# Hyberge/GPUFluidSimulation

Measured on AMD Instinct MI355X. Metric: Mvoxels/s per step (bimocq3D rising smoke), higher is better.
Workload: dtype f32

## Files before the change

gpufluidsimulation_amd/_lib.py:

```python
import ctypes as C
import os

HERE = os.path.dirname(os.path.abspath(__file__))
HIP_SO = os.path.join(HERE, "libbimocq_hip.so")
HOST_SO = os.path.join(HERE, "libbimocq_host.so")

VP = C.c_void_p
c_f, c_i, c_b, c_d = C.c_float, C.c_int, C.c_bool, C.c_double

_G = [c_f, c_i, c_i, c_i]

HIP_SIGS = {
    "gpu_solve_forward": (None, [VP] * 6 + _G + [c_f, c_f]),
    "gpu_solve_backwardDMC": (None, [VP] * 9 + _G + [c_f]),
    "gpu_advect_velocity": (None, [VP] * 9 + _G + [c_b]),
    "gpu_advect_vel_double": (None, [VP] * 12 + _G + [c_b, c_f]),
    "gpu_advect_field": (None, [VP] * 5 + _G + [c_b]),
    "gpu_advect_field_double": (None, [VP] * 8 + _G + [c_b, c_f]),
    "gpu_advect_vel_double_global": (None, [VP] * 12 + _G + [c_b, c_f]),
    "gpu_advect_field_double_global": (None, [VP] * 8 + _G + [c_b, c_f]),
    "gpu_accumulate_velocity": (None, [VP] * 9 + _G + [c_b, c_f]),
    "gpu_accumulate_field": (None, [VP] * 5 + _G + [c_b, c_f]),
    "gpu_estimate_distortion": (None, [VP] * 7 + _G),
    "gpu_add": (None, [VP, VP, c_f, c_i]),
# ... 28 lines not shown
    "fl_aux_end": (None, []),
    "fl_aux_join": (None, []),
    "fl_malloc_host": (VP, [C.c_size_t]),
    "fl_free_host": (None, [VP]),
    "fl_download_begin": (VP, [VP, VP, C.c_size_t]),
    "fl_download_wait": (c_i, [VP]),
    "fl_event_create": (VP, []),
    "fl_event_record": (None, [VP]),
    "fl_event_elapsed_ms": (c_f, [VP, VP]),
    "fl_event_destroy": (None, [VP]),
    "fl_last_error": (c_i, []),
    "fl_last_error_string": (C.c_char_p, []),
    "fl_clear_error": (None, []),
    "fl_compute_stream": (VP, []),
    "fl_set_option": (None, [c_i, c_i]),
    "fl_get_option": (c_i, [c_i]),
    "fl_jacobi_profile": (None, [C.POINTER(c_d), C.POINTER(C.c_longlong), C.POINTER(C.c_longlong)]),
    "fl_jacobi_kernel_name": (C.c_char_p, []),
    "fl_mg_smooth_kernel_name": (C.c_char_p, []),
    "fl_mg_fused_launches": (C.c_longlong, []),
    "fl_mg_residual_launches": (C.c_longlong, []),
    "fl_sparse_stats": (None, [C.POINTER(C.c_longlong), c_i]),
    "fl_sparse_stats_kind": (None, [c_i, C.POINTER(C.c_longlong), c_i]),
    "gpu_brick_flags": (c_i, [VP, VP, c_i, c_i, c_i, VP, C.POINTER(c_i)]),
    "gpu_init_maps": (None, [VP, VP, VP] + _G),
    "gpu_maps_quarter_safe": (c_i, [VP, VP, VP] + _G),
    "fl_map_guard_reset": (None, [c_i]),
    "fl_map_guard_read": (None, [C.POINTER(c_i)]),
    "fl_nonfinite_seen": (c_i, [c_i]),
    "gpu_solve_forward_hint": (None, [VP] * 6 + _G + [c_f, c_f, C.c_uint]),
    "gpu_solve_backwardDMC_hint": (None, [VP] * 9 + _G + [c_f, C.c_uint]),
    "fl_map_kernel_name": (C.c_char_p, [c_i]),
    "fl_map_kernels_seen": (c_i, [c_i]),
    "gpu_max_abs3": (c_f, [VP, VP, VP, c_i, c_i, c_i]),
    "gpu_divergence": (None, [VP] * 4 + [c_i, c_i, c_i, c_f]),
    "gpu_jacobi_sweeps": (c_i, [VP, VP, VP, c_i, c_i, c_i, c_i, c_f, c_f]),
    "gpu_gradient": (None, [VP] * 4 + [c_i, c_i, c_i, c_f]),
    "fl_comm_selftest": (c_i, []),
    "gpu_diffuse_sweeps": (c_i, [VP, VP, VP, c_i, c_i, c_i, c_i, c_f]),
    "gpu_max_field": (c_f, [VP, C.c_size_t]),
    "gpu_max_field_owned": (c_f, [VP, c_i, c_i, c_i]),
    "gpu_map_travel_z": (None, [VP, VP, c_f, c_i, c_i, c_i, C.POINTER(c_f)]),
    "gpu_smoothing_jacobi": (None, [VP, VP, VP, c_d, c_d, c_i, c_i, c_i, c_i]),
    "gpu_mgcg_slab_supported": (c_i, [c_i] * 8),
    "gpu_multi_grid_conjugate_gradient_slab": (None, [VP, VP, VP, VP] + [c_i] * 7 + [c_d]),
    "gpu_gradient_delta": (None, [VP] * 7 + [c_i, c_i, c_i, c_f]),
# ... 70 lines not shown
    "gpu_sample_particles": (c_i, [VP, c_i, c_i, c_i, c_f, c_f, c_f, c_f, VP, VP, VP, VP, C.c_long]),
    "gpu_seed_particles": (c_i, [VP] * 3 + [c_i] * 7 + [C.c_uint] + _G),
    "gpu_sort_particles": (c_i, [VP] * 8 + [C.c_long] + _G),
}

FL_OK, FL_ERR_NO_DEVICE, FL_ERR_HIP, FL_ERR_BAD_ARGUMENT, FL_ERR_UNSUPPORTED, FL_ERR_COMM = range(6)
FL_OPT_RESIDUAL_STRIDE, FL_OPT_SKIP_UNIT_BLEND, FL_OPT_JACOBI_VARIANT = 1, 2, 3
FL_OPT_PROFILE_JACOBI, FL_OPT_JACOBI_KCHUNK, FL_OPT_JACOBI_ROWS, FL_OPT_STRUCTURED_MAPS = 4, 5, 6, 7
FL_OPT_JACOBI_FUSE, FL_OPT_JACOBI_KCHUNK2, FL_OPT_MGCG_GRAPH, FL_OPT_FAST_LERP = 8, 9, 10, 11
FL_OPT_FUSED_HOUSEKEEPING = 12
FL_OPT_MAP_QUARTER_FP32 = 13
FL_OPT_MGCG_TILE = 14
FL_MAP_HINT_FINITE, FL_MAP_HINT_IDENTITY = 1, 2
FL_OPT_PROFILE_COMM = 15
FL_OPT_RESERVE_CUS = 16
FL_OPT_MGCG_BOTTOM = 17
FL_OPT_MGCG_FUSE = 20
FL_OPT_FIELD_WINDOW = 18
FL_OPT_COMM_CHECK = 19
FL_OPT_SKIP_EMPTY_BRICKS = 21
FL_OPT_DIAG_KCHUNK = 22
FL_OPT_RENDER_KCHUNK = 23
FL_OPT_CONFINE_KCHUNK = 24
STAT_NAMES = ("e2", "m2", "d2", "div_max", "rho", "rho_i", "rho_j", "rho_k", "T", "vort_max")
STAT_COUNT = len(STAT_NAMES)
LOAD_NAMES = ("px", "py", "pz", "mx", "my", "mz", "faces", "psum")
LOAD_COUNT = len(LOAD_NAMES)
MAX_BOUNDARIES = 16


class BimocqLibraryMissing(RuntimeError):
    pass


_hip = None


def hip_lib():
    global _hip
    if _hip is None:
        if not os.path.exists(HIP_SO):
            raise BimocqLibraryMissing(
                f"{HIP_SO} not found: build it with `make` (or __graft_entry__.build()); "
                "there is no CPU fallback for the product path")
        lib = C.CDLL(HIP_SO)
        for name, (res, args) in HIP_SIGS.items():
# ... 20 lines not shown
```

gpufluidsimulation_amd/csrc/bq_advect.hip:

```cpp
#include "bq_device.hip.h"
#include "bq_gather_op.hip.h"
#include "bq_host.h"
#include "bq_launch_geom.h"
#include "bq_obstacle.hip.h"
#include "bq_sparse.hip.h"

#include <algorithm>
#include <cstdint>
#include <type_traits>
#include <vector>

namespace bq {
inline namespace BQ_VARIANT {

#define BQ_IJK(nbi, nbj, nbk)                                   \
    const int i = blockIdx.x * 64 + threadIdx.x;                \
    const int j = blockIdx.y * 4 + threadIdx.y;                 \
    const int k = blockIdx.z + g.kw0;                           \
    if (i >= (nbi) || j >= (nbj) || k >= (nbk)) return;         \
    const int kg = k + g.koff;                                  \
    (void)kg;

#define BQ_IJK_WINDOW(ilo, ihi, jlo, jhi, klo, khi) BQ_IJK_WINDOW_AT((int)blockIdx.x, (int)blockIdx.y, (int)blockIdx.z, ilo, ihi, jlo, jhi, klo, khi)
#define BQ_IJK_WINDOW_AT(bx_, by_, bz_, ilo, ihi, jlo, jhi, klo, khi)                         \
// ... 98 lines not shown
    f3 pn = mk3(dmc_axis(pt.x, vl.x, ax, substep), dmc_axis(pt.y, vl.y, ay, substep), dmc_axis(pt.z, vl.z, az, substep));
    f3 r;
    if constexpr (IDIN) r = map_at_identity<P2>(in, sp, pn, g.ni, g.nj, g.nk);
    else r = map_at<P2>(in, sp, pn);
    size_t id = (size_t)i + (size_t)g.ni * j + (size_t)g.ni * g.nj * k;
    xo[id] = r.x; yo[id] = r.y; zo[id] = r.z;
    guard_map_values(guard, r, sp.h);
}

template <bool P2, bool PT, int SD>
__device__ __forceinline__ void mapped9(const Map3 &m, const Spacing &sp, const Nine &n, f3 c, int i, int j, int kl, f3 out[9])
{
    if constexpr (P2 && !PT && SD >= 0) {
        map9<SD == 1, SD == 2, SD == 3>(m, i, j, kl, out);
    } else {
        if (!PT) {
#pragma unroll
            for (int ii = 0; ii < 8; ii++) out[ii] = map_at<P2>(m, sp, nine_corner(n, c, ii));
        }
        out[8] = map_at<P2>(m, sp, c);
    }
}

template <bool P2, bool PT, int NF, bool GE1>
__device__ __forceinline__ void blend9_gather_w(const Field (&src)[NF], const Spacing &sp, f3 org, const f3 (&mp)[9],
                                                const float (&w)[NF], float (&sum)[NF], float (&value)[NF])
{
    if (!PT) {
#pragma unroll
        for (int ii = 0; ii < 8; ii++) {
            const Cell c = locate<P2, true>(src[0], sp, org, mp[ii]);
#pragma unroll
            for (int f = 0; f < NF; f++) sum[f] += w[f] * gather<GE1>(src[f], c);
        }
    }
    const Cell c = locate<P2, true>(src[0], sp, org, mp[8]);
#pragma unroll
    for (int f = 0; f < NF; f++) {
        value[f] = gather<GE1>(src[f], c);
        if (PT) sum[f] += w[f] * value[f];
    }
}
template <bool P2, bool PT, int NF, bool GE1>
__device__ __forceinline__ void blend9_gather(const Field (&src)[NF], const Spacing &sp, f3 org, const f3 (&mp)[9],
                                              float (&sum)[NF], float (&value)[NF])
{
    float w[NF];
#pragma unroll
    for (int f = 0; f < NF; f++) w[f] = PT ? 1.0f : 0.125f;
    blend9_gather_w<P2, PT, NF, GE1>(src, sp, org, mp, w, sum, value);
}
template <bool PT>
__device__ __forceinline__ bool wave_all_ge(const f3 (&mp)[9], float h)
{
    float m = fminf(mp[8].x, fminf(mp[8].y, mp[8].z));
    if (!PT) {
#pragma unroll
        for (int a9 = 0; a9 < 8; a9++) m = fminf(m, fminf(mp[a9].x, fminf(mp[a9].y, mp[a9].z)));
    }
// ... 107 lines not shown
}

__global__ __launch_bounds__(256) void unit_blend_kernel(float *field, Grid g, int dx, int dy, int dz)
{
    const int nbi = g.ni + dx, nbj = g.nj + dy, nbk = g.nk + dz;
    BQ_IJK(nbi, nbj, nbk)
    if (!(2 + dx < i && i < nbi - 3 && 2 + dy < j && j < nbj - 3 && 2 + dz < kg && kg < g.nkg + dz - 3)) return;
    size_t id = (size_t)i + (size_t)nbi * j + (size_t)nbi * nbj * k;
    field[id] = field[id] + 0.0f;
}

template <bool P2, bool PT, int SD, int NF, bool ID, bool Q4 = false, int SPARSE = 0>
__global__ __launch_bounds__(256, NF == 1 ? 7 : 6) void cumulate_kernel(CumulateArgs<NF> a,
                                                       const float *mx, const float *my, const float *mz,
                                                       Spacing sp, Grid g, int dx, int dy, int dz, MapTabs tabs, Sparse sps)
{
    static_assert(!SPARSE || (SD == 0 && !ID && kStaged<P2, PT, SD>), "the skip exists for unstaggered staged launches only");
    using Op = GatherOp<kOpCumulate>;
    constexpr int m = Op::margin;
    const int nbi = g.ni + dx, nbj = g.nj + dy, nbk = g.nk + dz;
    int bX = blockIdx.x, bY = blockIdx.y, bZ = blockIdx.z;
    if constexpr (SPARSE == 1) { if (*sps.word != sps.epoch) return; }
    if constexpr (SPARSE == 2) { if (!listed_block(sps, bX, bY, bZ)) return; }
    BQ_IJK_WINDOW_AT(bX, bY, bZ, m + dx, nbi - m - 1, m + dy, nbj - m - 1, m + dz, g.nkg + dz - m - 1)
    if (block_out) return;
    const float h = sp.h;
    Map3 map{make_field(mx, g.ni, g.nj, g.nk, g.koff), make_field(my, g.ni, g.nj, g.nk, g.koff), make_field(mz, g.ni, g.nj, g.nk, g.koff)};
    Nine n = nine_setup(h, dx, dy, dz);
    f3 lo = Op::lo(h), hi = Op::hi(h, g.ni, g.nj, g.nkg);
    f3 c = nine_centre(n, i, j, kg);
    const size_t id = (size_t)i + (size_t)nbi * j + (size_t)nbi * nbj * k;
    __shared__ float tile[kStaged<P2, PT, SD> && !ID && SPARSE != 1 ? 3 * kTile : 32];
    (void)tabs; (void)sps;
    if constexpr (SPARSE == 1) {
        const Field mf[3] = {map.x, map.y, map.z};
        float mn[3], mxv[3]; bool bad;
        float dst_own[NF];
#pragma unroll
        for (int f = 0; f < NF; f++) dst_own[f] = active ? a.dst[f][id] : 0.f;
        tile_range(mf, i0, j0, k, tile, m, nbi - m - 1, m, nbj - m - 1, mn, mxv, bad);
        const bool skip = taps_in_empty_bricks<P2>(sps, mn, mxv, bad, lo, hi, sp, nbi, nbj, nbk);
        count_block(sps, skip);
        if (!skip) { list_block(sps, bX + gridDim.x * (bY + gridDim.y * bZ)); return; }
        if (!active) return;
#pragma unroll
        for (int f = 0; f < NF; f++) {
// ... 16 lines not shown
            float s9[9];
            map9_component<0, 0, 0>(src, i, j, k, s9);
            float sum = 0.f;
#pragma unroll
            for (int ii = 0; ii < 8; ii++) sum += Op::weight(false, coeff) * s9[ii];
            a.dst[f][id] += Op::result(sum, s9[8], coeff, 0.f);
        }
        return;
    }
    f3 mp[9];
    if constexpr (kStaged<P2, PT, SD>) {
        const Field mf[3] = {map.x, map.y, map.z};
        stage_tiles<3>(mf, i0, j0, k, tile);
        if (!active) return;
        if constexpr (P2) map9_lds<SD == 1, SD == 2, SD == 3, Q4>(tile, mp);
        else map9_lds_tab<SD == 1, SD == 2, SD == 3>(tile, tabs, i, j, kg, mp);
    } else {
        if (!active) return;
        mapped9<P2, PT, SD>(map, sp, n, c, i, j, k, mp);
    }
    const bool ge1 = NF == 1 && wave_all_ge<PT>(mp, h);
#pragma unroll
    for (int a9 = 0; a9 < 9; a9++) mp[a9] = clamp3_ordered(mp[a9], lo, hi);
    Field src[NF];
    float sum[NF], value[NF], w[NF];
#pragma unroll
    for (int f = 0; f < NF; f++) {
        src[f] = make_field(a.src[f], nbi, nbj, nbk, g.koff);
        sum[f] = 0.f;
        w[f] = Op::weight(PT, a.coeff[f]);
    }
    if (NF == 1 && ge1) blend9_gather_w<P2, PT, NF, true>(src, sp, n.org, mp, w, sum, value);
    else                blend9_gather_w<P2, PT, NF, false>(src, sp, n.org, mp, w, sum, value);
#pragma unroll
    for (int f = 0; f < NF; f++) {
        a.dst[f][id] += Op::result(sum[f], value[f], a.coeff[f], 0.f);
    }
}

template <bool P2, int SD>
__global__ __launch_bounds__(256) void wall_fixup_kernel(const float *src, int src_nk, int src_koff,
                                                         const float *before, float *dst,
                                                         const float *mx, const float *my, const float *mz,
                                                         Spacing sp, Grid g, int dx, int dy, int dz, float coeff,
                                                         int face_axis, int face_index, int kw1)
{
    const int nbi = g.ni + dx, nbj = g.nj + dy, nbk = g.nk + dz;
    const int a = blockIdx.x * 64 + threadIdx.x, b = blockIdx.y * 4 + threadIdx.y;
    int i, j, k;
    if (face_axis == 0)      { i = face_index; j = a; k = b + g.kw0; }
    else if (face_axis == 1) { i = a; j = face_index; k = b + g.kw0; }
    else                     { i = a; j = b; k = face_index - g.koff; }
    if (i >= nbi || j >= nbj || k < g.kw0 || k >= kw1 || k >= nbk) return;
    const int kg = k + g.koff;
    using Op = GatherOp<kOpCumulate>;
    constexpr int om = Op::margin;
// ... 403 lines not shown
        kchunk = 32;
        while (kchunk > 8 && (long)gx * gy * ((planes + kchunk - 1) / kchunk) < 3L * 4 * rt().num_cus) kchunk /= 2;
    }
    const dim3 grid(gx, gy, (planes + kchunk - 1) / kchunk);
    hipStream_t st = rt().compute;
    const int kw1 = g.kw0 + planes;
    if (NF == 2 && KIND != kOpCumulate && sd != 0) return false;
#define BQ_MARCH(SDV, Q4V) gather_march_kernel<KIND, SDV, NF, Q4V><<<grid, kBlock, 0, st>>>(a, mx, my, mz, sp, g, dx, dy, dz, fused, kchunk, kw1)
#define BQ_MARCH_SD(Q4V)                                                                     \
    if constexpr (NF == 2 && KIND != kOpCumulate) { BQ_MARCH(0, Q4V); }                    \
    else switch (sd) { case 0: BQ_MARCH(0, Q4V); break; case 1: BQ_MARCH(1, Q4V); break; case 2: BQ_MARCH(2, Q4V); break; default: BQ_MARCH(3, Q4V); break; }
#ifdef BQ_FAST_LERP
    (void)q4;
    BQ_MARCH_SD(false)
#else
    if (q4) { BQ_MARCH_SD(true) } else { BQ_MARCH_SD(false) }
#endif
#undef BQ_MARCH_SD
#undef BQ_MARCH
    BQ_LAUNCH_CHECK("gather_march_kernel");
    return true;
}

template <int NF>
static Sparse brick_flags(bool eligible, int kind, const float *const (&src)[NF], int nbi, int nbj, int nbk, size_t nblocks, bool force = false)
{
    Runtime &r = rt();
    Sparse none{ nullptr, nullptr, nullptr, nullptr, 0, 0, 0 };
    if (!eligible || (!r.opt_skip_empty_bricks && !force) || r.compute_main) return none;
    const int nbx = (nbi + kBrick - 1) >> kBrickShift, nby = (nbj + kBrick - 1) >> kBrickShift, nbz = (nbk + kBrick - 1) >> kBrickShift;
    if (nby > 65535 || nbz > 65535) return none;
    const size_t nflags = (size_t)nbx * nby * nbz, list_at = (nflags + 255) & ~(size_t)255;
    const size_t need = list_at + 4 * (nblocks + 1);
    if (nblocks >= 0x7fffffffu) return none;
    if (!r.sparse_hdr) {
        if (!BQ_HIP(hipMalloc((void **)&r.sparse_hdr, 64))) { r.sparse_hdr = nullptr; return none; }
        if (!BQ_HIP(hipMemsetAsync(r.sparse_hdr, 0, 64, r.compute))) return none;
        r.sparse_epoch = 0;
    }
    if (need > r.sparse_cap) {
        if (r.sparse_flags) { (void)hipStreamSynchronize(r.compute); (void)hipFree(r.sparse_flags); r.sparse_flags = nullptr; r.sparse_cap = 0; }
        if (!BQ_HIP(hipMalloc((void **)&r.sparse_flags, need))) { r.sparse_flags = nullptr; return none; }
        r.sparse_cap = need;
    }
    if (r.sparse_epoch == 0x7fffffff) {
        if (!BQ_HIP(hipMemsetAsync(r.sparse_hdr, 0, 4, r.compute))) return none;
        r.sparse_epoch = 0;
    }
    const int epoch = ++r.sparse_epoch;
    BrickSrc<NF> bs;
    for (int f = 0; f < NF; f++) bs.p[f] = src[f];
    int *list = reinterpret_cast<int *>(r.sparse_flags + list_at);
    brick_flags_kernel<NF><<<dim3((nbi + 63) / 64, nby, nbz), kBlock, 0, r.compute>>>(bs, nbi, nbj, nbk, r.sparse_flags, r.sparse_hdr, epoch, list);
    if (!BQ_LAUNCH_CHECK("brick_flags_kernel")) return none;
    unsigned long long *stats = (r.opt_skip_empty_bricks == 2 || r.opt_skip_empty_bricks == 4) ? reinterpret_cast<unsigned long long *>(r.sparse_hdr + 2) + 2 * kind : nullptr;
    return Sparse{ r.sparse_flags, r.sparse_hdr, stats, list, epoch, nbx, nby };
}
static inline bool sparse_eligible(const Grid &g, int planes, int dx, int dy, int dz, bool staged)
{
    return staged && !dx && !dy && !dz && !rt().slab_on && g.koff == 0 && g.kw0 == 0 && planes == g.nk;
}

template <int KIND, int NF>
static auto plane_args(const GatherArgs<NF> &a)
{
    std::conditional_t<KIND == kOpAdvect, AdvectArgs<NF>, std::conditional_t<KIND == kOpCumulate, CumulateArgs<NF>, CompensateArgs<NF>>> k;
    for (int f = 0; f < NF; f++) {
        if constexpr (KIND == kOpAdvect) { k.field[f] = a.out[f]; k.init[f] = a.src[f]; }
        else if constexpr (KIND == kOpCumulate) { k.src[f] = a.src[f]; k.dst[f] = a.out[f]; k.coeff[f] = a.coeff[f]; }
        else { k.src[f] = a.src[f]; k.init[f] = a.aux[f]; k.err[f] = a.out[f]; }
    }
    return k;
}

template <int KIND, int NF>
static void gather_launch(const GatherArgs<NF> &a, const float *mx, const float *my, const float *mz,
                          Spacing sp, Grid g, int dx, int dy, int dz, bool pt, bool identity = false)
{
    using Op = GatherOp<KIND>;
    int planes;
    g = mk_grid_win(g.ni, g.nj, g.nk, dz, &planes);
    if (planes <= 0) return;
    const dim3 grid = grid_for(g.ni + dx, g.nj + dy, planes);
    hipStream_t st = rt().compute;
    const bool q4 = rt().opt_map_quarter_fp32 != 0;
    const int fused = Op::has_housekeeping ? rt().opt_fused_housekeeping : 0;
    const int sda = stag_axis(dx, dy, dz);
    if (!identity && march_launch<KIND, NF>(a, mx, my, mz, sp, g, planes, dx, dy, dz, pt, q4, fused)) return;
    int tab_ok = 0;
    const MapTabs tabs = (!sp.pow2 && !pt && rt().opt_structured_maps) ? map_tabs(sp, g, &tab_ok) : MapTabs{ nullptr, nullptr, 0 };
    const bool tabled = tabs.frac && tabs_cover(tab_ok, sda);
    const bool staged = !pt && rt().opt_structured_maps && (tabled || (sp.pow2 && !identity));
    const Sparse sps = brick_flags<NF>((KIND != kOpCumulate || rt().opt_skip_empty_bricks >= 3) && sparse_eligible(g, planes, dx, dy, dz, staged),
                                       Op::counter_slot, a.src, g.ni, g.nj, g.nk, (size_t)grid.x * grid.y * grid.z);
    const auto ka = plane_args<KIND>(a);
    dispatch_sd(sp.pow2, pt, sda, [&](auto P2, auto PT, auto SD) {
        constexpr bool p2 = decltype(P2)::value, ptc = decltype(PT)::value;
        constexpr int sd = decltype(SD)::value;
        auto launch = [&](auto ID, auto Q4, auto SPARSE) {
            constexpr bool idc = decltype(ID)::value, q4c = decltype(Q4)::value;
            constexpr int sparse = decltype(SPARSE)::value;
            if constexpr (KIND == kOpAdvect) advect_kernel<p2, ptc, sd, NF, q4c, sparse><<<grid, kBlock, 0, st>>>(ka, mx, my, mz, sp, g, dx, dy, dz, fused, tabs, sps);
            else if constexpr (KIND == kOpCumulate) cumulate_kernel<p2, ptc, sd, NF, idc, q4c, sparse><<<grid, kBlock, 0, st>>>(ka, mx, my, mz, sp, g, dx, dy, dz, tabs, sps);
            else compensate_kernel<p2, ptc, sd, NF, q4c, sparse><<<grid, kBlock, 0, st>>>(ka, mx, my, mz, sp, g, dx, dy, dz, fused, tabs, sps);
        };
        using T = std::true_type; using F = std::false_type;
        using Plain = std::integral_constant<int, 0>; using Classify = std::integral_constant<int, 1>; using Listed = std::integral_constant<int, 2>;
        if constexpr (sd == 0 && kStaged<p2, ptc, sd>) {
            if (sps.flags) {
                launch(F{}, F{}, Classify{});
                if (p2 && q4) launch(F{}, std::bool_constant<p2>{}, Listed{});
                else launch(F{}, F{}, Listed{});
                return;
            }
        }
        if constexpr (p2 && kStaged<p2, ptc, sd>) {
            if constexpr (KIND == kOpCumulate) { if (identity) { launch(T{}, F{}, Plain{}); return; } }
            if (q4) { launch(F{}, T{}, Plain{}); return; }
        }
        launch(F{}, F{}, Plain{});
    }, tabled);
    BQ_LAUNCH_CHECK(Op::kernel_name);
}

static void advect_comp(float *f, const float *init, const float *bx, const float *by, const float *bz,
                        Spacing sp, Grid g, int dx, int dy, int dz, bool pt)
{
    gather_launch<kOpAdvect, 1>(GatherArgs<1>{{init}, {f}, {nullptr}, {1.f}}, bx, by, bz, sp, g, dx, dy, dz, pt);
}
static void cumulate_comp(const float *src, float *dst, const float *mx, const float *my, const float *mz,
// ... 603 lines not shown

static void sparse_stats(int kind0, int kind1, long long out[2], int reset)
{
    if (!out) return;
    out[0] = out[1] = 0;
    Runtime &r = rt();
    if (!r.ready || !r.sparse_hdr) return;
    unsigned long long *host = (unsigned long long *)pinned(64);
    if (!host) return;
    hipStream_t st = r.compute;
    const size_t bytes = 16 * (size_t)(kind1 - kind0);
    unsigned long long *dev = reinterpret_cast<unsigned long long *>(r.sparse_hdr + 2) + 2 * kind0;
    if (!BQ_HIP(hipMemcpyAsync(host, dev, bytes, hipMemcpyDeviceToHost, st))) return;
    if (reset && !BQ_HIP(hipMemsetAsync(dev, 0, bytes, st))) return;
    if (!BQ_HIP(hipStreamSynchronize(st))) return;
    for (int k = 0; k < kind1 - kind0; k++) { out[0] += (long long)(host[2 * k] + host[2 * k + 1]); out[1] += (long long)host[2 * k + 1]; }
}
void fl_sparse_stats(long long out[2], int reset) { sparse_stats(0, 3, out, reset); }
void fl_sparse_stats_kind(int kind, long long out[2], int reset)
{
    if (kind < 0 || kind > 2) { latch(FL_ERR_BAD_ARGUMENT, "fl_sparse_stats_kind", "kind must be 0, 1 or 2"); return; }
    sparse_stats(kind, kind + 1, out, reset);
}

int gpu_brick_flags(const float *f1, const float *f2, int ni, int nj, int nk, unsigned char *flags_host, int *any_empty)
{
    if (!ensure_ready("gpu_brick_flags") || !dims_ok(ni, nj, nk, "gpu_brick_flags")) return -1;
    if (!f1 || !flags_host) { latch(FL_ERR_BAD_ARGUMENT, "gpu_brick_flags", "null pointer"); return -1; }
    Sparse s;
    if (f2) { const float *const src[2] = { f1, f2 }; s = brick_flags<2>(true, 0, src, ni, nj, nk, 0, true); }
    else { const float *const src[1] = { f1 }; s = brick_flags<1>(true, 0, src, ni, nj, nk, 0, true); }
    if (!s.flags) { latch(FL_ERR_UNSUPPORTED, "gpu_brick_flags", "no flag pass (an fl_aux_* section is open, or the allocation failed)"); return -1; }
    const size_t n = (size_t)s.nbx * s.nby * ((nk + kBrick - 1) >> kBrickShift);
    int *host = (int *)pinned(64);
    if (!host) return -1;
    hipStream_t st = rt().compute;
    if (!BQ_HIP(hipMemcpyAsync(flags_host, s.flags, n, hipMemcpyDeviceToHost, st)) ||
        !BQ_HIP(hipMemcpyAsync(host, s.word, 4, hipMemcpyDeviceToHost, st)) || !BQ_HIP(hipStreamSynchronize(st))) return -1;
    if (any_empty) *any_empty = host[0] == s.epoch;
    return (int)n;
}

const char *fl_map_kernel_name(int which) { return (which == 0 || which == 1) ? rt().map_kernel_name[which] : ""; }
int fl_map_kernels_seen(int reset)
{
    const int v = rt().map_kernels_seen;
// ... 44 lines not shown
```

gpufluidsimulation_amd/csrc/bq_host.h:

```cpp
#pragma once
#include <hip/hip_runtime.h>
#include <cmath>
#include <cstdint>
#include <cstdio>
#include <functional>
#include <initializer_list>
#include "../../include/bimocq_gpu.h"

namespace bq {

struct Runtime {
    bool        ready = false;
    int         device = -1;
    hipStream_t compute = nullptr;
    hipStream_t halo = nullptr;
    hipStream_t copy = nullptr;
    hipStream_t aux = nullptr, compute_main = nullptr;
    hipEvent_t  aux_fork = nullptr, aux_done = nullptr;
    bool        aux_pending = false;
    int         err = FL_OK;
    char        err_text[256] = {0};
    int         opt_residual_stride = 0;
    int         opt_skip_unit_blend = 1;
    int         opt_jacobi_variant = 0;
// ... 18 lines not shown
    int         device_cus = 0;
    int         num_cus = 256;
    int         opt_diag_kchunk = 0;
    int         opt_render_kchunk = 0;
    int         opt_confine_kchunk = 0;
    int         opt_jacobi_rows = 0;
    bool        win_on = false;
    int         win_k0 = 0, win_k1 = 0;
    bool        slab_on = false;
    int         slab_koff = 0, slab_nkg = 0, slab_own0 = 0, slab_own1 = 0, slab_nkl = 0;
    void  *scratch = nullptr;
    size_t scratch_bytes = 0;
    void  *pinned = nullptr;
    size_t pinned_bytes = 0;
    void  *halo_state = nullptr, *project_state = nullptr, *mgcg_state = nullptr;
    float *map_tab_dev = nullptr;
    float  map_tab_h = 0.f;
    int    map_tab_dims[3] = {0, 0, 0}, map_tab_stride = 0, map_tab_ok = 0;
    unsigned char *sparse_flags = nullptr;
    size_t sparse_cap = 0;
    int   *sparse_hdr = nullptr;
    int    sparse_epoch = 0;
    int    opt_skip_empty_bricks = 1;
    int    nonfinite_seen = 0;
    const char *map_kernel_name[2] = { "", "" };
    int    map_kernels_seen = 0;
    long long   mg_fused_launches = 0;
    long long   mg_residual_launches = 0;
    const char *mg_smooth_kernel = "";
};

Runtime &rt();
inline void slab_ctx(int nk, int &koff, int &nkg)
{
    const Runtime &r = rt();
    koff = r.slab_on ? r.slab_koff : 0;
    nkg = r.slab_on ? r.slab_nkg : nk;
}
void latch(int code, const char *what, const char *detail);
bool ensure_ready(const char *op);
void *scratch(size_t bytes);
void *pinned(size_t bytes);
bool comm_allreduce(void *dev, size_t count, bool is_double, bool is_max, hipStream_t st);
int  comm_ranks();
void mgcg_release_graph();
void mgcg_release_state(Runtime &r);
// ... 52 lines not shown
```

gpufluidsimulation_amd/csrc/bq_runtime.hip:

```cpp
#include "bq_host.h"
#include <cstdint>
#include <cstdio>
#include <cstdlib>
#include <cstring>
#include <mutex>
#include <vector>

namespace bq {

static Runtime g_default_rt;
static thread_local Runtime *t_current = nullptr;
static std::mutex g_mu;

static std::vector<Runtime *> g_live;
static std::once_flag g_exit_once;
static bool g_exiting = false;
static void note_live(Runtime *r, bool live)
{
    std::lock_guard<std::mutex> lk(g_mu);
    for (size_t a = 0; a < g_live.size(); a++)
        if (g_live[a] == r) { if (!live) g_live.erase(g_live.begin() + a); return; }
    if (live) g_live.push_back(r);
}

// ... 373 lines not shown
void fl_set_option(int option, int value)
{
    switch (option) {
    case FL_OPT_RESIDUAL_STRIDE: g_rt.opt_residual_stride = value < 0 ? 0 : value; break;
    case FL_OPT_SKIP_UNIT_BLEND: g_rt.opt_skip_unit_blend = (value == 1 || value == 2) ? value : 0; break;
    case FL_OPT_JACOBI_VARIANT:  g_rt.opt_jacobi_variant = value; break;
    case FL_OPT_PROFILE_JACOBI:  g_rt.opt_profile_jacobi = value ? 1 : 0; break;
    case FL_OPT_JACOBI_KCHUNK:   g_rt.opt_jacobi_kchunk = value < 0 ? 0 : value; break;
    case FL_OPT_JACOBI_ROWS:     g_rt.opt_jacobi_rows = value; break;
    case FL_OPT_STRUCTURED_MAPS: g_rt.opt_structured_maps = value ? 1 : 0; break;
    case FL_OPT_JACOBI_FUSE:     g_rt.opt_jacobi_fuse = value; break;
    case FL_OPT_JACOBI_KCHUNK2:  g_rt.opt_jacobi_kchunk2 = value < 0 ? 0 : value; break;
    case FL_OPT_MGCG_GRAPH:      g_rt.opt_mgcg_graph = value != 0; break;
    case FL_OPT_FAST_LERP:       g_rt.opt_fast_lerp = value != 0; break;
    case FL_OPT_FUSED_HOUSEKEEPING: g_rt.opt_fused_housekeeping = value & 15; break;
    case FL_OPT_MAP_QUARTER_FP32: g_rt.opt_map_quarter_fp32 = value != 0; break;
    case FL_OPT_MGCG_TILE:       g_rt.opt_mgcg_tile = value < 0 ? 0 : value; break;
    case FL_OPT_PROFILE_COMM:    g_rt.opt_profile_comm = value != 0; break;
    case FL_OPT_MGCG_BOTTOM:     g_rt.opt_mgcg_bottom = value != 0; break;
    case FL_OPT_MGCG_FUSE:       g_rt.opt_mgcg_fuse = value < 0 ? -1 : (value > 3 ? 3 : value); break;
    case FL_OPT_FIELD_WINDOW:    g_rt.opt_field_window = value < 0 ? -1 : value; break;
    case FL_OPT_COMM_CHECK:      g_rt.opt_comm_check = value != 0; break;
    case FL_OPT_SKIP_EMPTY_BRICKS: g_rt.opt_skip_empty_bricks = (value >= 1 && value <= 4) ? value : 0; break;
    case FL_OPT_DIAG_KCHUNK:     g_rt.opt_diag_kchunk = value < 0 ? -1 : value; break;
    case FL_OPT_RENDER_KCHUNK:   g_rt.opt_render_kchunk = value < 0 ? -1 : value; break;
    case FL_OPT_CONFINE_KCHUNK:  g_rt.opt_confine_kchunk = value < 0 ? -1 : value; break;
    case FL_OPT_RESERVE_CUS: {
        const int k = value < 0 ? 0 : value;
        if (k == g_rt.opt_reserve_cus) break;
        g_rt.opt_reserve_cus = k;
        if (!g_rt.ready) break;
        fl_sync();
        bq::mgcg_release_graph();
        (void)hipStreamDestroy(g_rt.compute);
        g_rt.compute = nullptr;
        if (!bq::create_compute_stream()) g_rt.ready = false;
        break;
    }
    default: bq::latch(FL_ERR_BAD_ARGUMENT, "fl_set_option", "unknown option");
    }
}

int fl_get_option(int option)
{
    switch (option) {
    case FL_OPT_RESIDUAL_STRIDE: return g_rt.opt_residual_stride;
    case FL_OPT_SKIP_UNIT_BLEND: return g_rt.opt_skip_unit_blend;
    case FL_OPT_JACOBI_VARIANT:  return g_rt.opt_jacobi_variant;
    case FL_OPT_PROFILE_JACOBI:  return g_rt.opt_profile_jacobi;
    case FL_OPT_JACOBI_KCHUNK:   return g_rt.opt_jacobi_kchunk;
    case FL_OPT_JACOBI_ROWS:     return g_rt.opt_jacobi_rows;
    case FL_OPT_STRUCTURED_MAPS: return g_rt.opt_structured_maps;
    case FL_OPT_JACOBI_FUSE:     return g_rt.opt_jacobi_fuse;
    case FL_OPT_JACOBI_KCHUNK2:  return g_rt.opt_jacobi_kchunk2;
    case FL_OPT_MGCG_GRAPH:      return g_rt.opt_mgcg_graph;
    case FL_OPT_FAST_LERP:       return g_rt.opt_fast_lerp;
    case FL_OPT_FUSED_HOUSEKEEPING: return g_rt.opt_fused_housekeeping;
    case FL_OPT_MAP_QUARTER_FP32: return g_rt.opt_map_quarter_fp32;
    case FL_OPT_MGCG_TILE:       return g_rt.opt_mgcg_tile;
    case FL_OPT_PROFILE_COMM:    return g_rt.opt_profile_comm;
    case FL_OPT_MGCG_BOTTOM:     return g_rt.opt_mgcg_bottom;
    case FL_OPT_MGCG_FUSE:       return g_rt.opt_mgcg_fuse;
    case FL_OPT_FIELD_WINDOW:    return g_rt.opt_field_window;
    case FL_OPT_COMM_CHECK:      return g_rt.opt_comm_check;
    case FL_OPT_SKIP_EMPTY_BRICKS: return g_rt.opt_skip_empty_bricks;
    case FL_OPT_DIAG_KCHUNK:     return g_rt.opt_diag_kchunk;
    case FL_OPT_RENDER_KCHUNK:   return g_rt.opt_render_kchunk;
    case FL_OPT_CONFINE_KCHUNK:  return g_rt.opt_confine_kchunk;
    case FL_OPT_RESERVE_CUS:     return g_rt.opt_reserve_cus;
    default: return -1;
    }
}

}
```

gpufluidsimulation_amd/csrc/bq_sparse.hip.h:

```cpp
#pragma once
#include "bq_device.hip.h"

namespace bq {
inline namespace BQ_VARIANT {

constexpr int kBrick = 8, kBrickShift = 3;

struct Sparse {
    const unsigned char *flags;
    const int *word;
    unsigned long long *stats;
    int *list;
    int epoch, nbx, nby;
};
template <int NF> struct BrickSrc { const float *p[NF]; };

template <int NF>
__global__ __launch_bounds__(256) void brick_flags_kernel(BrickSrc<NF> s, int nx, int ny, int nz,
                                                          unsigned char *flags, int *word, int epoch, int *list)
{
    __shared__ unsigned part[4][8];
    const int lane = threadIdx.x, wv = threadIdx.y;
    const int x = blockIdx.x * 64 + lane, y0 = blockIdx.y * kBrick, z0 = blockIdx.z * kBrick;
    unsigned acc = 0u;
// ... 125 lines not shown
}

__device__ __forceinline__ void list_block(const Sparse &s, int b)
{
    if (threadIdx.x == 0 && threadIdx.y == 0) s.list[1 + atomicAdd(s.list, 1)] = b;
}
__device__ __forceinline__ bool listed_block(const Sparse &s, int &bX, int &bY, int &bZ)
{
    if (*s.word != s.epoch) return true;
    const int b = bX + gridDim.x * (bY + gridDim.y * bZ);
    if (b >= s.list[0]) return false;
    const int e = s.list[1 + b];
    bX = e % (int)gridDim.x;
    const int t = e / (int)gridDim.x;
    bY = t % (int)gridDim.y; bZ = t / (int)gridDim.y;
    return true;
}

__device__ __forceinline__ void count_block(const Sparse &s, bool skipped)
{
    if (s.stats && threadIdx.x == 0 && threadIdx.y == 0) atomicAdd(s.stats + (skipped ? 1 : 0), 1ull);
}

}
}
```

include/bimocq_gpu.h:

```cpp
#ifndef BIMOCQ_GPU_H
#define BIMOCQ_GPU_H

#include <stddef.h>
#ifndef __cplusplus
#include <stdbool.h>
#endif

#ifdef __cplusplus
extern "C" {
#endif

#define LEVEL_COUNT 6
struct SCoarseLevelInfo {
    int ni, nj, nk;
    int number;
    double alpha;
    double beta;
    double *b;
    double *x;
    double *r;
};
#ifndef __cplusplus
typedef struct SCoarseLevelInfo SCoarseLevelInfo;
#endif
// ... 144 lines not shown
    FL_OPT_RESIDUAL_STRIDE = 1,
    FL_OPT_SKIP_UNIT_BLEND = 2,
    FL_OPT_JACOBI_VARIANT  = 3,
    FL_OPT_PROFILE_JACOBI  = 4,
    FL_OPT_JACOBI_KCHUNK   = 5,
    FL_OPT_JACOBI_ROWS     = 6,
    FL_OPT_STRUCTURED_MAPS = 7,
    FL_OPT_JACOBI_FUSE     = 8,
    FL_OPT_JACOBI_KCHUNK2  = 9,
    FL_OPT_MGCG_GRAPH      = 10,
    FL_OPT_FUSED_HOUSEKEEPING = 12,
    FL_OPT_FAST_LERP       = 11,
    FL_OPT_MGCG_TILE       = 14,
    FL_OPT_PROFILE_COMM    = 15,
    FL_OPT_RESERVE_CUS     = 16,
    FL_OPT_MGCG_BOTTOM     = 17,
    FL_OPT_FIELD_WINDOW    = 18,
    FL_OPT_COMM_CHECK      = 19,
    FL_OPT_MGCG_FUSE       = 20,
    FL_OPT_SKIP_EMPTY_BRICKS = 21,
    FL_OPT_DIAG_KCHUNK     = 22,
    FL_OPT_RENDER_KCHUNK   = 23,
    FL_OPT_CONFINE_KCHUNK = 24,
    FL_OPT_MAP_QUARTER_FP32 = 13
};
void fl_set_option(int option, int value);
int  fl_get_option(int option);
void fl_jacobi_profile(double *total_ms, long long *launches, long long *sweeps);
const char *fl_jacobi_kernel_name(void);
const char *fl_mg_smooth_kernel_name(void);
long long fl_mg_fused_launches(void);
long long fl_mg_residual_launches(void);
void fl_sparse_stats(long long out[2], int reset);
void fl_sparse_stats_kind(int kind, long long out[2], int reset);
int gpu_brick_flags(const float *f1, const float *f2, int ni, int nj, int nk, unsigned char *flags_host, int *any_empty);

int  fl_nonfinite_seen(int reset);
int  gpu_maps_quarter_safe(const float *x, const float *y, const float *z, float h, int ni, int nj, int nk);
void fl_map_guard_reset(int which);
void fl_map_guard_read(int ok[2]);
void gpu_init_maps(float *x, float *y, float *z, float h, int ni, int nj, int nk);
enum { FL_MAP_HINT_FINITE = 1, FL_MAP_HINT_IDENTITY = 2 };
void gpu_solve_forward_hint(float *u, float *v, float *w, float *x_fwd, float *y_fwd, float *z_fwd,
                            float h, int ni, int nj, int nk, float cfldt, float dt, unsigned hints);
void gpu_solve_backwardDMC_hint(float *u, float *v, float *w, float *x_in, float *y_in, float *z_in,
                                float *x_out, float *y_out, float *z_out,
                                float h, int ni, int nj, int nk, float substep, unsigned hints);
const char *fl_map_kernel_name(int which);
int  fl_map_kernels_seen(int reset);
float gpu_max_abs3(const float *u, const float *v, const float *w, int ni, int nj, int nk);
void gpu_divergence(const float *u, const float *v, const float *w, float *div,
                    int ni, int nj, int nk, float halfrdx);
int  gpu_jacobi_sweeps(float *p, const float *div, float *p_temp,
                       int ni, int nj, int nk, int sweeps, float alpha, float beta);
void gpu_gradient(float *u, float *v, float *w, const float *p,
                  int ni, int nj, int nk, float halfrdx);
void gpu_gradient_delta(float *u, float *v, float *w, const float *p, float *du, float *dv, float *dw,
// ... 240 lines not shown
```

Baseline: 1614.

## Skip cumulate-advection waves whose interpolation taps only hit empty bricks

Adds a per-wavefront sparsity test for the accumulate (cumulate) advection kernel. A new cell-flag kernel dilates the brick occupancy flags so that each trilinear footprint can be checked. Waves whose nine mapped sample positions all fall in empty cells skip the gathers and write a zero contribution. Blocks that are entirely empty are then handled by a second listed-block launch. It also stashes two of the mapped positions in shared memory to relieve register pressure and splits multi-field gathers per field. In exchange it costs an extra flag kernel, a second launch and extra flag reads per thread.

```diff
diff --git a/gpufluidsimulation_amd/_lib.py b/gpufluidsimulation_amd/_lib.py
--- a/gpufluidsimulation_amd/_lib.py
+++ b/gpufluidsimulation_amd/_lib.py
@@ -74,6 +74,7 @@
     "fl_mg_residual_launches": (C.c_longlong, []),
     "fl_sparse_stats": (None, [C.POINTER(C.c_longlong), c_i]),
     "fl_sparse_stats_kind": (None, [c_i, C.POINTER(C.c_longlong), c_i]),
+    "fl_sparse_wave_stats": (None, [C.POINTER(C.c_longlong), c_i]),
     "gpu_brick_flags": (c_i, [VP, VP, c_i, c_i, c_i, VP, C.POINTER(c_i)]),
     "gpu_init_maps": (None, [VP, VP, VP] + _G),
     "gpu_maps_quarter_safe": (c_i, [VP, VP, VP] + _G),
@@ -190,6 +191,7 @@
 FL_OPT_DIAG_KCHUNK = 22
 FL_OPT_RENDER_KCHUNK = 23
 FL_OPT_CONFINE_KCHUNK = 24
+FL_OPT_SKIP_EMPTY_TAPS = 25
 STAT_NAMES = ("e2", "m2", "d2", "div_max", "rho", "rho_i", "rho_j", "rho_k", "T", "vort_max")
 STAT_COUNT = len(STAT_NAMES)
 LOAD_NAMES = ("px", "py", "pz", "mx", "my", "mz", "faces", "psum")
diff --git a/gpufluidsimulation_amd/csrc/bq_advect.hip b/gpufluidsimulation_amd/csrc/bq_advect.hip
--- a/gpufluidsimulation_amd/csrc/bq_advect.hip
+++ b/gpufluidsimulation_amd/csrc/bq_advect.hip
@@ -144,19 +144,37 @@
     }
 }
 
-template <bool P2, bool PT, int NF, bool GE1>
+template <bool P2, bool PT, int NF, bool GE1, int STASHED = 0>
 __device__ __forceinline__ void blend9_gather_w(const Field (&src)[NF], const Spacing &sp, f3 org, const f3 (&mp)[9],
-                                                const float (&w)[NF], float (&sum)[NF], float (&value)[NF])
-{
+                                                const float (&w)[NF], float (&sum)[NF], float (&value)[NF], float *stash = nullptr)
+{
+    static_assert(STASHED == 0 || !PT, "point mode has one position");
+    auto pos = [&](int ii) -> f3 {
+        if constexpr (STASHED > 0) {
+            if (ii >= 9 - STASHED) {
+                if (ii == 9 - STASHED) asm volatile("" ::: "memory");
+                const int t = 3 * (ii - (9 - STASHED));
+                return mk3(stash[256 * t], stash[256 * (t + 1)], stash[256 * (t + 2)]);
+            }
+        }
+        return mp[ii];
+    };
+    if constexpr (STASHED > 0) {
+#pragma unroll
+        for (int t = 0; t < STASHED; t++) {
+            stash[256 * (3 * t)] = mp[9 - STASHED + t].x; stash[256 * (3 * t + 1)] = mp[9 - STASHED + t].y; stash[256 * (3 * t + 2)] = mp[9 - STASHED + t].z;
+        }
+        asm volatile("" ::: "memory");
+    }
     if (!PT) {
 #pragma unroll
         for (int ii = 0; ii < 8; ii++) {
-            const Cell c = locate<P2, true>(src[0], sp, org, mp[ii]);
+            const Cell c = locate<P2, true>(src[0], sp, org, pos(ii));
 #pragma unroll
             for (int f = 0; f < NF; f++) sum[f] += w[f] * gather<GE1>(src[f], c);
         }
     }
-    const Cell c = locate<P2, true>(src[0], sp, org, mp[8]);
+    const Cell c = locate<P2, true>(src[0], sp, org, pos(8));
 #pragma unroll
     for (int f = 0; f < NF; f++) {
         value[f] = gather<GE1>(src[f], c);
@@ -310,6 +328,7 @@
     int bX = blockIdx.x, bY = blockIdx.y, bZ = blockIdx.z;
     if constexpr (SPARSE == 1) { if (*sps.word != sps.epoch) return; }
     if constexpr (SPARSE == 2) { if (!listed_block(sps, bX, bY, bZ)) return; }
+    if constexpr (SPARSE == 3) { if (*sps.word != sps.epoch) return; }
     BQ_IJK_WINDOW_AT(bX, bY, bZ, m + dx, nbi - m - 1, m + dy, nbj - m - 1, m + dz, g.nkg + dz - m - 1)
     if (block_out) return;
     const float h = sp.h;
@@ -372,6 +391,22 @@
     const bool ge1 = NF == 1 && wave_all_ge<PT>(mp, h);
 #pragma unroll
     for (int a9 = 0; a9 < 9; a9++) mp[a9] = clamp3_ordered(mp[a9], lo, hi);
+    if constexpr (SPARSE == 3) {
+        static_assert(P2, "the wave test locates its cells by the power-of-two form of locate()");
+        const bool skip = !wave_taps_may_read(sps, sp, mp);
+        count_wave(sps, skip);
+        if (skip) {
+#pragma unroll
+            for (int f = 0; f < NF; f++) {
+                const float w = Op::weight(PT, a.coeff[f]);
+                float sum = 0.f;
+#pragma unroll
+                for (int ii = 0; ii < (PT ? 1 : 8); ii++) sum += w * 0.f;
+                a.dst[f][id] += Op::result(sum, 0.f, a.coeff[f], 0.f);
+            }
+            return;
+        }
+    }
     Field src[NF];
     float sum[NF], value[NF], w[NF];
 #pragma unroll
@@ -380,8 +415,28 @@
         sum[f] = 0.f;
         w[f] = Op::weight(PT, a.coeff[f]);
     }
+    if constexpr (SPARSE == 3 && NF == 1) {
+        constexpr int stashed = 2;
+        __shared__ float late[3 * stashed * 256];
+        float *mine = late + threadIdx.x + 64 * threadIdx.y;
+        if (ge1) blend9_gather_w<P2, PT, NF, true, stashed>(src, sp, n.org, mp, w, sum, value, mine);
+        else     blend9_gather_w<P2, PT, NF, false, stashed>(src, sp, n.org, mp, w, sum, value, mine);
+    } else if constexpr (SPARSE == 3) {
+#pragma unroll
+        for (int f = 0; f < NF; f++) {
+#pragma unroll
+            for (int a9 = 0; a9 < 9; a9++) asm volatile("" : "+v"(mp[a9].x), "+v"(mp[a9].y), "+v"(mp[a9].z));
+            const f3 (&p)[9] = mp;
+            const Field s1[1] = { src[f] };
+            const float w1[1] = { w[f] };
+            float sum1[1] = { 0.f }, value1[1];
+            blend9_gather_w<P2, PT, 1, false>(s1, sp, n.org, p, w1, sum1, value1);
+            sum[f] = sum1[0]; value[f] = value1[0];
+        }
+    } else {
     if (NF == 1 && ge1) blend9_gather_w<P2, PT, NF, true>(src, sp, n.org, mp, w, sum, value);
     else                blend9_gather_w<P2, PT, NF, false>(src, sp, n.org, mp, w, sum, value);
+    }
 #pragma unroll
     for (int f = 0; f < NF; f++) {
         a.dst[f][id] += Op::result(sum[f], value[f], a.coeff[f], 0.f);
@@ -831,6 +886,12 @@
     return true;
 }
 
+constexpr size_t kSparseHdrBytes = 128;
+static inline size_t sparse_cells_at(size_t nflags, size_t nblocks)
+{
+    const size_t list_at = (nflags + 255) & ~(size_t)255;
+    return (list_at + 4 * (nblocks + 1) + 255) & ~(size_t)255;
+}
 template <int NF>
 static Sparse brick_flags(bool eligible, int kind, const float *const (&src)[NF], int nbi, int nbj, int nbk, size_t nblocks, bool force = false)
 {
@@ -840,11 +901,12 @@
     const int nbx = (nbi + kBrick - 1) >> kBrickShift, nby = (nbj + kBrick - 1) >> kBrickShift, nbz = (nbk + kBrick - 1) >> kBrickShift;
     if (nby > 65535 || nbz > 65535) return none;
     const size_t nflags = (size_t)nbx * nby * nbz, list_at = (nflags + 255) & ~(size_t)255;
-    const size_t need = list_at + 4 * (nblocks + 1);
+    const CellDims cd = cell_dims(nbi, nbj, nbk);
+    const size_t need = sparse_cells_at(nflags, nblocks) + (size_t)cd.ncx * cd.ncy * cd.ncz;
     if (nblocks >= 0x7fffffffu) return none;
     if (!r.sparse_hdr) {
-        if (!BQ_HIP(hipMalloc((void **)&r.sparse_hdr, 64))) { r.sparse_hdr = nullptr; return none; }
-        if (!BQ_HIP(hipMemsetAsync(r.sparse_hdr, 0, 64, r.compute))) return none;
+        if (!BQ_HIP(hipMalloc((void **)&r.sparse_hdr, kSparseHdrBytes))) { r.sparse_hdr = nullptr; return none; }
+        if (!BQ_HIP(hipMemsetAsync(r.sparse_hdr, 0, kSparseHdrBytes, r.compute))) return none;
         r.sparse_epoch = 0;
     }
     if (need > r.sparse_cap) {
@@ -864,6 +926,20 @@
     if (!BQ_LAUNCH_CHECK("brick_flags_kernel")) return none;
     unsigned long long *stats = (r.opt_skip_empty_bricks == 2 || r.opt_skip_empty_bricks == 4) ? reinterpret_cast<unsigned long long *>(r.sparse_hdr + 2) + 2 * kind : nullptr;
     return Sparse{ r.sparse_flags, r.sparse_hdr, stats, list, epoch, nbx, nby };
+}
+static Sparse cell_flags(const Sparse &s, int nbi, int nbj, int nbk, size_t nblocks)
+{
+    Runtime &r = rt();
+    const Sparse none{ nullptr, nullptr, nullptr, nullptr, 0, 0, 0 };
+    const int nbz = (nbk + kBrick - 1) >> kBrickShift;
+    const CellDims cd = cell_dims(nbi, nbj, nbk);
+    const size_t ncells = (size_t)cd.ncx * cd.ncy * cd.ncz;
+    if (ncells >= 0x7fffffffu) return none;
+    unsigned char *cells = r.sparse_flags + sparse_cells_at((size_t)s.nbx * s.nby * nbz, nblocks);
+    cell_flags_kernel<<<dim3((unsigned)((ncells + 3) / 4)), kBlock, 0, r.compute>>>(s.flags, cells, nbi, nbj, nbk);
+    if (!BQ_LAUNCH_CHECK("cell_flags_kernel")) return none;
+    unsigned long long *stats = (r.opt_skip_empty_bricks == 2 || r.opt_skip_empty_bricks == 4) ? reinterpret_cast<unsigned long long *>(r.sparse_hdr + 16) : nullptr;
+    return Sparse{ cells, s.word, stats, nullptr, s.epoch, cd.ncx, cd.ncy };
 }
 static inline bool sparse_eligible(const Grid &g, int planes, int dx, int dy, int dz, bool staged)
 {
@@ -900,8 +976,13 @@
     const MapTabs tabs = (!sp.pow2 && !pt && rt().opt_structured_maps) ? map_tabs(sp, g, &tab_ok) : MapTabs{ nullptr, nullptr, 0 };
     const bool tabled = tabs.frac && tabs_cover(tab_ok, sda);
     const bool staged = !pt && rt().opt_structured_maps && (tabled || (sp.pow2 && !identity));
-    const Sparse sps = brick_flags<NF>((KIND != kOpCumulate || rt().opt_skip_empty_bricks >= 3) && sparse_eligible(g, planes, dx, dy, dz, staged),
-                                       Op::counter_slot, a.src, g.ni, g.nj, g.nk, (size_t)grid.x * grid.y * grid.z);
+    const bool eligible = sparse_eligible(g, planes, dx, dy, dz, staged);
+    const int skip_opt = rt().opt_skip_empty_bricks;
+    const bool wave = KIND == kOpCumulate && sp.pow2 && rt().opt_skip_empty_taps && (skip_opt == 1 || skip_opt == 2) && eligible;
+    const size_t nblocks = (size_t)grid.x * grid.y * grid.z;
+    Sparse sps = brick_flags<NF>((KIND != kOpCumulate || skip_opt >= 3 || wave) && eligible, Op::counter_slot, a.src, g.ni, g.nj, g.nk, nblocks);
+    const Sparse bricks = sps;
+    if (wave && sps.flags) sps = cell_flags(sps, g.ni, g.nj, g.nk, nblocks);
     const auto ka = plane_args<KIND>(a);
     dispatch_sd(sp.pow2, pt, sda, [&](auto P2, auto PT, auto SD) {
         constexpr bool p2 = decltype(P2)::value, ptc = decltype(PT)::value;
@@ -915,6 +996,17 @@
         };
         using T = std::true_type; using F = std::false_type;
         using Plain = std::integral_constant<int, 0>; using Classify = std::integral_constant<int, 1>; using Listed = std::integral_constant<int, 2>;
+        if constexpr (KIND == kOpCumulate && p2 && sd == 0 && kStaged<p2, ptc, sd>) {
+            if (wave && sps.flags) {
+                using WaveTest = std::integral_constant<int, 3>;
+                if (q4) launch(F{}, T{}, WaveTest{});
+                else launch(F{}, F{}, WaveTest{});
+                sps = bricks;
+                if (q4) launch(F{}, T{}, Listed{});
+                else launch(F{}, F{}, Listed{});
+                return;
+            }
+        }
         if constexpr (sd == 0 && kStaged<p2, ptc, sd>) {
             if (sps.flags) {
                 launch(F{}, F{}, Classify{});
@@ -1564,6 +1656,21 @@
     if (kind < 0 || kind > 2) { latch(FL_ERR_BAD_ARGUMENT, "fl_sparse_stats_kind", "kind must be 0, 1 or 2"); return; }
     sparse_stats(kind, kind + 1, out, reset);
 }
+void fl_sparse_wave_stats(long long out[2], int reset)
+{
+    if (!out) return;
+    out[0] = out[1] = 0;
+    Runtime &r = rt();
+    if (!r.ready || !r.sparse_hdr) return;
+    unsigned long long *host = (unsigned long long *)pinned(64);
+    if (!host) return;
+    hipStream_t st = r.compute;
+    unsigned long long *dev = reinterpret_cast<unsigned long long *>(r.sparse_hdr + 16);
+    if (!BQ_HIP(hipMemcpyAsync(host, dev, 16, hipMemcpyDeviceToHost, st))) return;
+    if (reset && !BQ_HIP(hipMemsetAsync(dev, 0, 16, st))) return;
+    if (!BQ_HIP(hipStreamSynchronize(st))) return;
+    out[0] = (long long)(host[0] + host[1]); out[1] = (long long)host[1];
+}
 
 int gpu_brick_flags(const float *f1, const float *f2, int ni, int nj, int nk, unsigned char *flags_host, int *any_empty)
 {
diff --git a/gpufluidsimulation_amd/csrc/bq_host.h b/gpufluidsimulation_amd/csrc/bq_host.h
--- a/gpufluidsimulation_amd/csrc/bq_host.h
+++ b/gpufluidsimulation_amd/csrc/bq_host.h
@@ -64,6 +64,7 @@
     int   *sparse_hdr = nullptr;
     int    sparse_epoch = 0;
     int    opt_skip_empty_bricks = 1;
+    int    opt_skip_empty_taps = 1;
     int    nonfinite_seen = 0;
     const char *map_kernel_name[2] = { "", "" };
     int    map_kernels_seen = 0;
diff --git a/gpufluidsimulation_amd/csrc/bq_runtime.hip b/gpufluidsimulation_amd/csrc/bq_runtime.hip
--- a/gpufluidsimulation_amd/csrc/bq_runtime.hip
+++ b/gpufluidsimulation_amd/csrc/bq_runtime.hip
@@ -419,6 +419,7 @@
     case FL_OPT_FIELD_WINDOW:    g_rt.opt_field_window = value < 0 ? -1 : value; break;
     case FL_OPT_COMM_CHECK:      g_rt.opt_comm_check = value != 0; break;
     case FL_OPT_SKIP_EMPTY_BRICKS: g_rt.opt_skip_empty_bricks = (value >= 1 && value <= 4) ? value : 0; break;
+    case FL_OPT_SKIP_EMPTY_TAPS: g_rt.opt_skip_empty_taps = value != 0; break;
     case FL_OPT_DIAG_KCHUNK:     g_rt.opt_diag_kchunk = value < 0 ? -1 : value; break;
     case FL_OPT_RENDER_KCHUNK:   g_rt.opt_render_kchunk = value < 0 ? -1 : value; break;
     case FL_OPT_CONFINE_KCHUNK:  g_rt.opt_confine_kchunk = value < 0 ? -1 : value; break;
@@ -461,6 +462,7 @@
     case FL_OPT_FIELD_WINDOW:    return g_rt.opt_field_window;
     case FL_OPT_COMM_CHECK:      return g_rt.opt_comm_check;
     case FL_OPT_SKIP_EMPTY_BRICKS: return g_rt.opt_skip_empty_bricks;
+    case FL_OPT_SKIP_EMPTY_TAPS: return g_rt.opt_skip_empty_taps;
     case FL_OPT_DIAG_KCHUNK:     return g_rt.opt_diag_kchunk;
     case FL_OPT_RENDER_KCHUNK:   return g_rt.opt_render_kchunk;
     case FL_OPT_CONFINE_KCHUNK:  return g_rt.opt_confine_kchunk;
diff --git a/gpufluidsimulation_amd/csrc/bq_sparse.hip.h b/gpufluidsimulation_amd/csrc/bq_sparse.hip.h
--- a/gpufluidsimulation_amd/csrc/bq_sparse.hip.h
+++ b/gpufluidsimulation_amd/csrc/bq_sparse.hip.h
@@ -171,5 +171,58 @@
     if (s.stats && threadIdx.x == 0 && threadIdx.y == 0) atomicAdd(s.stats + (skipped ? 1 : 0), 1ull);
 }
 
-}
-}
+struct CellDims { int ncx, ncy, ncz; };
+__host__ __device__ inline CellDims cell_dims(int nx, int ny, int nz)
+{
+    return CellDims{ (nx >> kBrickShift) + 1, (ny >> kBrickShift) + 1, (nz >> kBrickShift) + 1 };
+}
+
+__global__ __launch_bounds__(256) void cell_flags_kernel(const unsigned char *flags, unsigned char *cells, int nx, int ny, int nz)
+{
+    const CellDims d = cell_dims(nx, ny, nz);
+    const int c = __builtin_amdgcn_readfirstlane((int)(blockIdx.x * 4 + threadIdx.y));
+    if (c >= d.ncx * d.ncy * d.ncz) return;
+    const int cx = c % d.ncx, t = c / d.ncx, cy = t % d.ncy, cz = t / d.ncy;
+    int x0 = cx << kBrickShift, x1 = min(x0 + kBrick - 1, nx) + 1;
+    int y0 = cy << kBrickShift, y1 = min(y0 + kBrick - 1, ny) + 1;
+    int z0 = cz << kBrickShift, z1 = min(z0 + kBrick - 1, nz) + 1;
+    if (x1 > nx - 1) { x0 = 0; x1 = nx - 1; y1 += 1; }
+    if (y1 > ny - 1) { y0 = 0; y1 = ny - 1; z1 += 1; }
+    z1 = min(z1, nz - 1);
+    bool occupied = false;
+    if (z0 <= z1) {
+        const int nbx = (nx + kBrick - 1) >> kBrickShift, nby = (ny + kBrick - 1) >> kBrickShift;
+        const int bx0 = x0 >> kBrickShift, by0 = y0 >> kBrickShift, bz0 = z0 >> kBrickShift;
+        const int wx = (x1 >> kBrickShift) - bx0 + 1, wy = (y1 >> kBrickShift) - by0 + 1, wz = (z1 >> kBrickShift) - bz0 + 1;
+        for (int e = (int)threadIdx.x; e < wx * wy * wz; e += 64) {
+            const int ex = e % wx, r = e / wx, ey = r % wy, ez = r / wy;
+            occupied |= flags[(size_t)(bx0 + ex) + (size_t)nbx * ((by0 + ey) + (size_t)nby * (bz0 + ez))] != 0;
+        }
+    }
+    const bool any = __any(occupied);
+    if (threadIdx.x == 0) cells[c] = any ? 1 : 0;
+}
+
+__device__ __forceinline__ bool wave_taps_may_read(const Sparse &s, const Spacing &sp, const f3 (&mp)[9])
+{
+    unsigned char fl[9];
+#pragma unroll
+    for (int a9 = 0; a9 < 9; a9++) {
+        const int i = floor_to_int(mp[a9].x * sp.inv_h), j = floor_to_int(mp[a9].y * sp.inv_h), k = floor_to_int(mp[a9].z * sp.inv_h);
+        fl[a9] = s.flags[(unsigned)((i >> kBrickShift) + __mul24(s.nbx, (j >> kBrickShift) + __mul24(s.nby, k >> kBrickShift)))];
+    }
+    unsigned acc = 0u;
+#pragma unroll
+    for (int a9 = 0; a9 < 9; a9++) acc |= fl[a9];
+    return __any(acc != 0u);
+}
+
+__device__ __forceinline__ void count_wave(const Sparse &s, bool skipped)
+{
+    if (!s.stats) return;
+    const unsigned long long live = __ballot(1);
+    if (__lane_id() == (unsigned)(__ffsll((long long)live) - 1)) atomicAdd(s.stats + (skipped ? 1 : 0), 1ull);
+}
+
+}
+}
diff --git a/include/bimocq_gpu.h b/include/bimocq_gpu.h
--- a/include/bimocq_gpu.h
+++ b/include/bimocq_gpu.h
@@ -190,6 +190,7 @@
     FL_OPT_DIAG_KCHUNK     = 22,
     FL_OPT_RENDER_KCHUNK   = 23,
     FL_OPT_CONFINE_KCHUNK = 24,
+    FL_OPT_SKIP_EMPTY_TAPS = 25,
     FL_OPT_MAP_QUARTER_FP32 = 13
 };
 void fl_set_option(int option, int value);
@@ -201,6 +202,7 @@
 long long fl_mg_residual_launches(void);
 void fl_sparse_stats(long long out[2], int reset);
 void fl_sparse_stats_kind(int kind, long long out[2], int reset);
+void fl_sparse_wave_stats(long long out[2], int reset);
 int gpu_brick_flags(const float *f1, const float *f2, int ni, int nj, int nk, unsigned char *flags_host, int *any_empty);
 
 int  fl_nonfinite_seen(int reset);
```

Measured after the change: 1653, median of 6. +2.4%, better.
